# qway/nerfmeshes

Measured on AMD Instinct MI355X. Metric: rendered rays/sec (64+128 samples, 8x256 MLP), lego scene geometry, higher is better.
Workload: dtype f32; 1 GPU; nerf-synthetic lego: 8x256 coarse+fine MLP, 64 coarse + 128 fine samples, 800x800 view per step per rank, bounds [2,6], seeded weights/orbit poses; chunk_rays=65536, parallelism=single GPU

## Files before the change

### include/nerfmeshes_hip.h

```cpp
#ifndef NERFMESHES_HIP_H
#define NERFMESHES_HIP_H

#include <stdint.h>

#ifdef __cplusplus
extern "C" {
#endif

#define NM_ABI_VERSION 6

const char* nm_last_error(void);
int nm_abi_version(void);
int nm_device_count(void);

typedef struct nm_mlp_desc {
    int32_t num_layers;
    int32_t hidden_size;
    int32_t skip_step;
    int32_t num_encoding_fn_xyz;
    int32_t num_encoding_fn_dir;
    int32_t include_input_xyz;
    int32_t include_input_dir;
    int32_t use_viewdirs;
} nm_mlp_desc;
// ... 3 lines not shown
    const float* const* layers_xyz_w; const float* const* layers_xyz_b;
    const float* layers_dir0_w;       const float* layers_dir0_b;
    const float* fc_alpha_w;          const float* fc_alpha_b;
    const float* fc_rgb_w;            const float* fc_rgb_b;
    const float* fc_feat_w;           const float* fc_feat_b;
    const float* freq_xyz;
    const float* freq_dir;
} nm_mlp_weights;

typedef struct nm_mlp nm_mlp;

int nm_mlp_create(const nm_mlp_desc* desc, const nm_mlp_weights* h_weights, int device, nm_mlp** out);

enum { NM_PREC_F32 = 0, NM_PREC_BF16X3 = 1 };
enum { NM_KERNEL_GENERIC = 0x100 };
int nm_mlp_create_ex(const nm_mlp_desc* desc, const nm_mlp_weights* host_weights, int device, int precision, nm_mlp** out);
int nm_mlp_precision(const nm_mlp* mlp);
void nm_mlp_destroy(nm_mlp* mlp);
int nm_mlp_kernel_variant(const nm_mlp* mlp, int* waves_per_workgroup);
int64_t nm_mlp_flops_per_sample(const nm_mlp* mlp, int density_only);

int nm_mlp_profile_enable(int on);
int nm_mlp_profile_read(int64_t* launches, double* total_ms, double* total_flops);

int nm_mlp_sample_points(nm_mlp* mlp, const float* d_points, const float* d_dirs, int64_t n,
                         float* d_radiance, void* stream);

int nm_mlp_eval_rays(nm_mlp* mlp, const float* d_origins, int origins_per_ray, const float* d_dirs,
                     const float* d_t, int64_t rays, int32_t samples, float* d_radiance, void* stream);

int nm_mlp_grid_query(nm_mlp* mlp, const float* d_ax0, const float* d_ax1, const float* d_ax2,
                      int32_t n0, int32_t n1, int32_t n2, int64_t first, int64_t count,
                      int32_t density_only, float* d_out, void* stream);

int nm_mlp_sample_density(nm_mlp* mlp, const float* d_points, int64_t n, float* d_sigma, void* stream);

int64_t nm_mlp_density_grad_workspace_bytes(const nm_mlp* mlp, int64_t n);
int nm_mlp_density_grad(nm_mlp* mlp, const float* d_points, int64_t n, void* d_workspace, int64_t workspace_bytes,
                        float* d_grad , void* stream);


int nm_ray_bundle(const float* h_c2w, int32_t height, int32_t width, float focal, int64_t first,
                  int64_t count, float* d_dirs, float* h_origin, void* stream);

typedef struct nm_view {
    float c2w[12];
// ... 308 lines not shown
```

### nerfmeshes_amd/_lib.py

```python
import ctypes as C
import os

LIB_PATH = os.path.join(os.path.dirname(os.path.abspath(__file__)), "csrc", "libnerfmeshes_hip.so")

c_float_p = C.POINTER(C.c_float)
c_void_p = C.c_void_p


class MlpDesc(C.Structure):
    _fields_ = [(n, C.c_int32) for n in ("num_layers", "hidden_size", "skip_step", "num_encoding_fn_xyz",
                                         "num_encoding_fn_dir", "include_input_xyz", "include_input_dir",
                                         "use_viewdirs")]


class MlpWeights(C.Structure):
    _fields_ = [("layer1_w", c_void_p), ("layer1_b", c_void_p),
                ("layers_xyz_w", C.POINTER(c_void_p)), ("layers_xyz_b", C.POINTER(c_void_p)),
                ("layers_dir0_w", c_void_p), ("layers_dir0_b", c_void_p),
                ("fc_alpha_w", c_void_p), ("fc_alpha_b", c_void_p),
                ("fc_rgb_w", c_void_p), ("fc_rgb_b", c_void_p),
                ("fc_feat_w", c_void_p), ("fc_feat_b", c_void_p),
                ("freq_xyz", c_void_p), ("freq_dir", c_void_p)]


# ... 27 lines not shown

class RenderCfg(C.Structure):
    _fields_ = [("num_coarse", C.c_int32), ("num_fine", C.c_int32), ("lindisp", C.c_int32),
                ("white_background", C.c_int32), ("training", C.c_int32), ("attenuation_threshold", C.c_float)]


class View(C.Structure):
    _fields_ = [("c2w", C.c_float * 12), ("height", C.c_int32), ("width", C.c_int32), ("focal", C.c_double),
                ("use_ndc", C.c_int32), ("ndc_near", C.c_double)]


SIGNATURES = {
    "nm_last_error": (C.c_char_p, []),
    "nm_abi_version": (C.c_int, []),
    "nm_device_count": (C.c_int, []),
    "nm_mlp_create": (C.c_int, [C.POINTER(MlpDesc), C.POINTER(MlpWeights), C.c_int, C.POINTER(c_void_p)]),
    "nm_mlp_create_ex": (C.c_int, [C.POINTER(MlpDesc), C.POINTER(MlpWeights), C.c_int, C.c_int, C.POINTER(c_void_p)]),
    "nm_mlp_precision": (C.c_int, [c_void_p]),
    "nm_mlp_destroy": (None, [c_void_p]),
    "nm_mlp_kernel_variant": (C.c_int, [c_void_p, C.POINTER(C.c_int)]),
    "nm_mlp_flops_per_sample": (C.c_int64, [c_void_p, C.c_int]),
    "nm_mlp_profile_enable": (C.c_int, [C.c_int]),
    "nm_mlp_profile_read": (C.c_int, [C.POINTER(C.c_int64), C.POINTER(C.c_double), C.POINTER(C.c_double)]),
    "nm_mlp_sample_points": (C.c_int, [c_void_p, c_void_p, c_void_p, C.c_int64, c_void_p, c_void_p]),
    "nm_mlp_sample_density": (C.c_int, [c_void_p, c_void_p, C.c_int64, c_void_p, c_void_p]),
    "nm_mlp_density_grad_workspace_bytes": (C.c_int64, [c_void_p, C.c_int64]),
    "nm_mlp_density_grad": (C.c_int, [c_void_p, c_void_p, C.c_int64, c_void_p, C.c_int64, c_void_p, c_void_p]),
    "nm_mlp_eval_rays": (C.c_int, [c_void_p, c_void_p, C.c_int, c_void_p, c_void_p, C.c_int64, C.c_int32, c_void_p,
                                   c_void_p]),
    "nm_mlp_grid_query": (C.c_int, [c_void_p, c_void_p, c_void_p, c_void_p, C.c_int32, C.c_int32, C.c_int32,
                                    C.c_int64, C.c_int64, C.c_int32, c_void_p, c_void_p]),
    "nm_ray_bundle": (C.c_int, [c_float_p, C.c_int32, C.c_int32, C.c_float, C.c_int64, C.c_int64, c_void_p,
                                c_float_p, c_void_p]),
    "nm_coarse_intervals": (C.c_int, [c_void_p, c_void_p, c_void_p, C.c_int, C.c_int, C.c_int64, C.c_int32,
                                      c_void_p, c_void_p]),
    "nm_composite": (C.c_int, [c_void_p, c_void_p, c_void_p, C.c_int64, C.c_int32, C.c_float, C.c_int, C.c_int,
                               C.POINTER(BundleOut), c_void_p]),
    "nm_sample_pdf": (C.c_int, [c_void_p, c_void_p, c_void_p, C.c_int64, C.c_int32, C.c_int32, c_void_p, c_void_p]),
    "nm_render_workspace_bytes": (C.c_int64, [C.c_int64, C.c_int32, C.c_int32]),
    "nm_render_rays": (C.c_int, [c_void_p, c_void_p, C.POINTER(RenderCfg), c_void_p, C.c_int, c_void_p, c_void_p,
                                 c_void_p, C.c_int, c_void_p, c_void_p, C.c_int64, c_void_p, C.POINTER(BundleOut),
                                 C.POINTER(BundleOut), c_void_p]),
    "nm_render_view": (C.c_int, [c_void_p, c_void_p, C.POINTER(RenderCfg), C.POINTER(View), C.c_int64, C.c_int64, c_void_p,
                                 c_void_p, C.c_int, c_void_p, c_void_p, c_void_p, C.POINTER(BundleOut),
                                 C.POINTER(BundleOut), c_void_p]),
    "nm_view_rays": (C.c_int, [C.POINTER(View), C.c_int64, C.c_int64, c_void_p, c_void_p, c_void_p]),
# ... 148 lines not shown
```

### nerfmeshes_amd/csrc/mlp_api.hip

```cpp
#include <cstring>
#include <map>
#include <mutex>
#include <utility>
#include <vector>

#include "nm_internal.h"
#include "mlp_device_g.h"
#include "nerf_layerwise.h"

namespace nm {

static thread_local std::string g_error;
void set_error(const std::string& msg) { g_error = msg; }

int ensure_dynamic_lds(const void* kernel, int bytes) {
    NM_REQUIRE(bytes <= 160 * 1024, "LDS budget exceeded");
    static std::mutex lock;
    static std::map<std::pair<int, const void*>, int> have;
    int dev = 0;
    NM_HIP_CHECK(hipGetDevice(&dev));
    std::lock_guard<std::mutex> guard(lock);
    int& cur = have[{dev, kernel}];
    if (cur < bytes) {
        NM_HIP_CHECK(hipFuncSetAttribute(kernel, hipFuncAttributeMaxDynamicSharedMemorySize, bytes));
// ... 105 lines not shown
                       static_cast<float*>(m->d_blob), n, m->d_check);
    if (m->precision == NM_PREC_BF16X3) {
        const int64_t nb = (int64_t)m->b3_units * 512;
        hipLaunchKernelGGL(gather_parameters<true>, dim3((unsigned)((nb + 255) / 256)), dim3(256), 0, stream, m->d_index_b3, ptrs,
                           m->d_tmp_b3, nb, static_cast<unsigned long long*>(nullptr));
        hipLaunchKernelGGL(split_b3_kernel, dim3((unsigned)((m->b3_units * 64 + 255) / 256)), dim3(256), 0, stream,
                           m->d_tmp_b3, static_cast<uint4*>(m->d_stream_b3), (int64_t)m->b3_units);
    }
    NM_HIP_CHECK(hipGetLastError());
    ++m->refresh_count;
    return 0;
}

MlpArgs ray_mode_args(const nm_mlp* m, const float* d_origins, int origins_per_ray, const float* d_dirs, const float* d_t, int64_t rays,
                      int32_t samples, float* d_radiance) {
    MlpArgs a = m->base;
    a.mode = MODE_RAYS;
    a.a = d_origins; a.b = d_dirs; a.c = d_t;
    a.origins_per_ray = origins_per_ray; a.samples = samples;
    a.n = rays * samples; a.out = d_radiance;
    return a;
}

struct ProfRec { hipEvent_t start, stop; double flops; int slot, device; double skip_flops; };
static bool g_prof_on = false;
static std::vector<ProfRec> g_prof;
constexpr int PROF_SKIP_SLOTS = 1 << 20;
struct ProfSkips { uint32_t* d = nullptr; int used = 0; };
static std::vector<ProfSkips> g_prof_skips;

static int launch_mlp_timed(const nm_mlp* m, const MlpArgs& a, int density_only, hipStream_t stream) {
    if (!density_only && !m->desc.use_viewdirs) density_only = 2;
    auto launch = [&]() { return m->lw ? layerwise_forward(const_cast<nm_mlp*>(m), a, density_only, stream) : launch_mlp(m, a, density_only, stream); };
    if (!g_prof_on || a.n <= 0) return launch();
    ProfRec r;
    NM_HIP_CHECK(hipEventCreate(&r.start));
    NM_HIP_CHECK(hipEventCreate(&r.stop));
    r.flops = (double)a.n * (double)(density_only == 1 ? m->flops_density : m->flops_full);
    r.slot = -1; r.device = -1; r.skip_flops = 0;
    MlpArgs counted = a;
    if (a.skip_empty && !density_only && !m->lw) {
        ProfSkips* ps = m->device >= 0 && m->device < (int)g_prof_skips.size() ? &g_prof_skips[m->device] : nullptr;
        if (ps && ps->d && ps->used < PROF_SKIP_SLOTS) {
            r.slot = ps->used++; r.device = m->device;
            r.skip_flops = (double)m->plan->wg_samples * (double)(m->flops_full - m->flops_density);
            counted.skip_count = ps->d + r.slot;
        } else {
            counted.skip_empty = 0;
        }
    }
    NM_HIP_CHECK(hipEventRecord(r.start, stream));
    const int rc = m->lw ? launch() : launch_mlp(m, counted, density_only, stream);
    NM_HIP_CHECK(hipEventRecord(r.stop, stream));
    g_prof.push_back(r);
    return rc;
}

static int validate_create(const nm_mlp_desc& d, const nm_mlp_weights* w, int precision, bool force_generic) {
    NM_REQUIRE(precision == NM_PREC_F32 || precision == NM_PREC_BF16X3, "unknown precision");
    NM_REQUIRE(!force_generic || precision == NM_PREC_F32, "NM_KERNEL_GENERIC goes with NM_PREC_F32");
    NM_REQUIRE(d.use_viewdirs == 0 || d.use_viewdirs == 1, "use_viewdirs is 0 or 1");
    const bool no_view = d.use_viewdirs == 0;
    NM_REQUIRE(!no_view || precision == NM_PREC_F32, "use_viewdirs=0 networks run in fp32 only");
    NM_REQUIRE(d.num_layers >= 2 && d.num_layers <= 32, "num_layers out of range");
    NM_REQUIRE(d.skip_step >= 1, "skip_step must be >= 1");
    NM_REQUIRE(d.hidden_size >= 1 && d.num_encoding_fn_xyz >= 0 && d.num_encoding_fn_dir >= 0, "negative network dimension");
    NM_REQUIRE(no_view || d.hidden_size >= 2, "hidden_size = 1 with view directions: layers_dir[0] would have hidden_size // 2 = 0 rows");
    NM_REQUIRE(d.num_encoding_fn_xyz > 0 || d.include_input_xyz,
               "the xyz encoding is empty (num_encoding_fn_xyz = 0 without include_input_xyz): layer1 would have no input");
// ... 129 lines not shown
}

}

using namespace nm;

extern "C" {

const char* nm_last_error(void) { return g_error.c_str(); }
int nm_abi_version(void) { return NM_ABI_VERSION; }
int nm_device_count(void) {
    int n = 0;
    if (hipGetDeviceCount(&n) != hipSuccess) return -1;
    return n;
}

int nm_mlp_profile_enable(int on) {
    if (on && g_prof_skips.empty()) {
        int count = 0;
        NM_HIP_CHECK(hipGetDeviceCount(&count));
        std::vector<ProfSkips> slots(count);
        for (int dev = 0; dev < count; ++dev) {
            DeviceGuard guard(dev);
            NM_HIP_CHECK(hipMalloc(&slots[dev].d, PROF_SKIP_SLOTS * sizeof(uint32_t)));
            NM_HIP_CHECK(hipMemset(slots[dev].d, 0, PROF_SKIP_SLOTS * sizeof(uint32_t)));
        }
        g_prof_skips.swap(slots);
    }
    g_prof_on = on != 0;
    return 0;
}

int nm_mlp_profile_read(int64_t* launches, double* total_ms, double* total_flops) {
    double ms = 0, fl = 0;
    std::vector<uint32_t> skips;
    for (ProfRec& r : g_prof) {
        NM_HIP_CHECK(hipEventSynchronize(r.stop));
        float t = 0;
        NM_HIP_CHECK(hipEventElapsedTime(&t, r.start, r.stop));
        ms += t; fl += r.flops;
        (void)hipEventDestroy(r.start); (void)hipEventDestroy(r.stop);
    }
    for (int dev = 0; dev < (int)g_prof_skips.size(); ++dev) {
        ProfSkips& ps = g_prof_skips[dev];
        if (ps.used == 0) continue;
        DeviceGuard guard(dev);
        skips.resize(ps.used);
        NM_HIP_CHECK(hipMemcpy(skips.data(), ps.d, skips.size() * sizeof(uint32_t), hipMemcpyDeviceToHost));
        NM_HIP_CHECK(hipMemset(ps.d, 0, skips.size() * sizeof(uint32_t)));
        for (const ProfRec& r : g_prof)
            if (r.slot >= 0 && r.device == dev) fl -= (double)skips[r.slot] * r.skip_flops;
        ps.used = 0;
    }
    if (launches) *launches = (int64_t)g_prof.size();
    if (total_ms) *total_ms = ms;
    if (total_flops) *total_flops = fl;
    g_prof.clear();
    return 0;
}

int nm_mlp_create(const nm_mlp_desc* desc, const nm_mlp_weights* w, int device, nm_mlp** out) {
    return nm_mlp_create_ex(desc, w, device, NM_PREC_F32, out);
}

int nm_mlp_precision(const nm_mlp* m) { return m ? m->precision : -1; }

int nm_mlp_create_ex(const nm_mlp_desc* desc, const nm_mlp_weights* w, int device, int precision, nm_mlp** out) {
    NM_REQUIRE(desc && w && out, "null argument");
    const bool force_generic = (precision & NM_KERNEL_GENERIC) != 0;
    precision &= ~NM_KERNEL_GENERIC;
    const nm_mlp_desc& d = *desc;
    if (int rc = validate_create(d, w, precision, force_generic)) return rc;
    const MlpPlan* plan = nullptr;
    if (int rc = choose_plan(d, precision, force_generic, &plan)) return rc;
    LwNet* lw_net = nullptr;
    if (plan == &g_layerwise_plan) {
// ... 159 lines not shown
    return launch_mlp_timed(m, a, 0, static_cast<hipStream_t>(stream));
}

int nm_mlp_sample_density(nm_mlp* m, const float* d_points, int64_t n, float* d_sigma, void* stream) {
    NM_REQUIRE(m && d_points && d_sigma && n >= 0, "bad argument");
    NM_REQUIRE(m->precision == NM_PREC_F32, "sample_density: geometry is fp32 by contract (bf16x3 handle)");
    MlpArgs a = m->base;
    a.mode = MODE_POINTS;
    a.a = d_points; a.b = d_points; a.c = nullptr;
    a.n = n; a.out = d_sigma;
    return launch_mlp_timed(m, a, 1, static_cast<hipStream_t>(stream));
}

int nm_mlp_eval_rays(nm_mlp* m, const float* d_origins, int origins_per_ray, const float* d_dirs, const float* d_t,
                     int64_t rays, int32_t samples, float* d_radiance, void* stream) {
    NM_REQUIRE(m && d_origins && d_dirs && d_t && d_radiance && rays >= 0 && samples > 0, "bad argument");
    return launch_mlp_timed(m, ray_mode_args(m, d_origins, origins_per_ray, d_dirs, d_t, rays, samples, d_radiance), 0, static_cast<hipStream_t>(stream));
}

}

namespace nm {
int nm_mlp_eval_render_internal(nm_mlp* m, const RayGen* gen, const float* d_origins, int origins_per_ray, const float* d_dirs,
                                const float* d_t, int64_t rays, int32_t samples, float* d_radiance, hipStream_t stream) {
    NM_REQUIRE(m && (gen || (d_origins && d_dirs)) && d_t && d_radiance && rays >= 0 && samples > 0, "bad argument");
    MlpArgs a = ray_mode_args(m, d_origins, origins_per_ray, d_dirs, d_t, rays, samples, d_radiance);
    if (gen) {
        a.mode = MODE_VIEW;
        a.a = nullptr; a.b = nullptr;
        a.gen = *gen;
    }
    a.skip_empty = 1;
    return launch_mlp_timed(m, a, 0, stream);
}
}

extern "C" {

int nm_mlp_grid_query(nm_mlp* m, const float* d_ax0, const float* d_ax1, const float* d_ax2, int32_t n0, int32_t n1,
                      int32_t n2, int64_t first, int64_t count, int32_t density_only, float* d_out, void* stream) {
    NM_REQUIRE(m && d_ax0 && d_ax1 && d_ax2 && d_out, "bad argument");
    NM_REQUIRE(n0 > 0 && n1 > 0 && n2 > 0 && first >= 0 && count >= 0 &&
               first + count <= (int64_t)n0 * n1 * n2, "grid range");
    MlpArgs a = m->base;
    a.mode = MODE_GRID;
    a.a = d_ax0; a.b = d_ax1; a.c = d_ax2;
    a.n1 = n1; a.n2 = n2; a.first = first;
    a.n = count; a.out = d_out;
    return launch_mlp_timed(m, a, density_only ? 1 : 0, static_cast<hipStream_t>(stream));
}

}
```

### nerfmeshes_amd/csrc/mlp_device_r3.h

```cpp
#pragma once
#include "mlp_device.h"

namespace nm {

struct NextChunks {
    const char* s0; int b0;
    const char* s1; int b1;
};

template <int NT, int KS1, int KS2, int NW, int LDSBUF, int KCH>
__device__ __forceinline__ void gemm_stage3(f32x4 (&acc)[NT], const float (&b1)[KS1],
                                            const float (&b2)[(KS2 > 0 ? KS2 : 1)], const char* gw,
                                            const NextChunks nx, char* lds, int& slot, f32x4 (&carry)[2],
                                            int wave, int lane) {
    constexpr int KS = KS1 + KS2;
    constexpr int NCH = (KS + KCH - 1) / KCH;
    constexpr int NB = NT / 4;
    constexpr int STEP_BYTES = NT * 256;
    static_assert(NT % 4 == 0 && NB >= 1, "tile count");
    static_assert(NCH >= 2, "every stage must span at least two chunks (DMA runs two chunks ahead)");
    f32x4 ab[3];
    ab[0] = carry[0];
    ab[1] = carry[1];
#pragma unroll
// ... 60 lines not shown
    const int64_t wg_iters = mlp_wg_iters(args, NW * 16);
    auto hidden_next = [](const char* p) {
        return NextChunks{p, KCH * N::STEP, p + KCH * N::STEP, (N::KH - KCH < KCH ? N::KH - KCH : KCH) * N::STEP};
    };
    auto enc_next = [](const char* p, bool on) {
        return NextChunks{p, on ? KCH * N::STEP : 0, p + KCH * N::STEP,
                          on ? (N::EX - KCH < KCH ? N::EX - KCH : KCH) * N::STEP : 0};
    };
    auto dir_next = [](const char* p) { return NextChunks{p, KCH * N::STEPD, p + KCH * N::STEPD, KCH * N::STEPD}; };

    int slot = 0;
    f32x4 carry[2];
    if ((int64_t)blockIdx.x < wg_iters) {
        const NextChunks first = enc_next(args.wstream, true);
        stream_to_lds<NW>(first.s0, lds, first.b0, wave, lane);
        stream_to_lds<NW>(first.s1, lds + N::LDSBUF, first.b1, wave, lane);
    }
    __syncthreads();
    carry[0] = *reinterpret_cast<const f32x4*>(lds + lane * 16);
    carry[1] = *reinterpret_cast<const f32x4*>(lds + lane * 16 + 1024);

    int64_t next_it = 0;
    int turn = 0;
    for (int64_t it = blockIdx.x; it < wg_iters; it = SKIP ? next_it : it + gridDim.x) {
        bool has_next = !SKIP && it + gridDim.x < wg_iters;
        int64_t sample = (it * NW + wave) * 16 + col;
        bool valid = sample < args.n;
        if (SKIP && args.ray_tiles) {
            const uint32_t depth_slots = (uint32_t)args.samples >> 4;
            const uint32_t block = (uint32_t)it / depth_slots;
            const int64_t ray_first = ((int64_t)block * NW + wave) * args.samples;
            sample = ray_first + (((uint32_t)it - block * depth_slots) << 4) + col;
            valid = ray_first < args.n;
        }
        const int64_t sidx = valid ? sample : args.n - 1;
        const SamplePD smp = fetch_sample(args, sidx);
        const float p[3] = {smp.px, smp.py, smp.pz}, d[3] = {smp.dx, smp.dy, smp.dz};
        const float dummy[1] = {0.0f};
        float encx[N::EX];
        encode<FX, N::EX>(encx, p, args.bands_xyz, g);
        NextChunks wrap = enc_next(args.wstream, has_next);

        f32x4 acc[N::NT];
        float in[N::KH];
        const char* gw = args.wstream;
        load_bias<N::NT>(acc, lds_bias, g);
        gemm_stage3<N::NT, N::EX, 0, NW, N::LDSBUF, KCH>(acc, encx, dummy, gw, hidden_next(gw + N::EX * N::STEP), lds, slot, carry, wave, lane);
        gw += N::EX * N::STEP;
        acc_to_operand<N::NT, false>(acc, in);
        if (SKIP && threadIdx.x == 0) lds_claim[turn] = atomicAdd(args.tile_queue, 1u);

        float sigma = 0.0f;
        bool empty_tile = false;
        const int trunk_iters = density_only ? num_layers - 1 : num_layers;
#pragma unroll 1
        for (int i = 0; i < trunk_iters; ++i) {
            const bool is_feat = i == num_layers - 1;
            if (is_feat) sigma = alpha_gemv<H>(in, lds_walpha, g) + tail_bias[0];
            if (SKIP && is_feat) {
                const int epoch = (int)it + 1;
                const bool dense = valid && !(sigma <= 0.0f);
                if (dense) *lds_vote = epoch;
                __syncthreads();
                empty_tile = __builtin_amdgcn_readfirstlane(*lds_vote) != epoch;
                next_it = (int64_t)gridDim.x + (uint32_t)__builtin_amdgcn_readfirstlane((int)lds_claim[turn]);
                turn ^= 1;
                has_next = next_it < wg_iters;
                wrap = enc_next(args.wstream, has_next);
                if (empty_tile) break;
            }
            const bool skip = !is_feat && ((args.skip_mask >> i) & 1u);
            const bool last_density = density_only && i == num_layers - 2;
            load_bias<N::NT>(acc, lds_bias + H * (1 + i), g);
            {
                const char* after = gw + N::KH * N::STEP;
                NextChunks nx = hidden_next(after);
                if (skip) nx = enc_next(after, true);
                else if (is_feat) nx = dir_next(after);
                else if (last_density) nx = wrap;
                gemm_stage3<N::NT, N::KH, 0, NW, N::LDSBUF, KCH>(acc, in, dummy, gw, nx, lds, slot, carry, wave, lane);
                gw = after;
            }
            if (skip) {
                const char* after = gw + N::EX * N::STEP;
                const NextChunks nx = last_density ? wrap : hidden_next(after);
                gemm_stage3<N::NT, N::EX, 0, NW, N::LDSBUF, KCH>(acc, encx, dummy, gw, nx, lds, slot, carry, wave, lane);
                gw = after;
            }
// ... 60 lines not shown
```

### nerfmeshes_amd/csrc/nerf_mlp.hip

```cpp
#include <iterator>
#include <vector>

#include "nm_internal.h"
#include "mlp_device.h"
#include "mlp_device_r3.h"
#include "mlp_device_b3.h"
#include "mlp_device_g.h"

namespace nm {

template <int H, int FX, int FD, int NW, int KCH>
static MlpPlan make_plan() {
    return MlpPlan{H, FX, FD, NW, KCH, 0, 2 * Net<H, FX, FD, KCH>::LDSBUF, &mlp_kernel<H, FX, FD, NW, KCH, false>,
                   NW * 16, 8 / NW, &mlp_kernel<H, FX, FD, NW, KCH, false, true>, 0, nullptr, nullptr};
}

template <int H, int FX, int FD, int NW, int KCH, bool SKIP = true>
static MlpPlan make_plan3() {
    return MlpPlan{H, FX, FD, NW, KCH, 0, 3 * Net<H, FX, FD, KCH>::LDSBUF, &mlp_kernel3<H, FX, FD, NW, KCH>,
                   NW * 16, 8 / NW, &mlp_kernel3<H, FX, FD, NW, KCH, true>, 0, nullptr, nullptr,
                   SKIP ? &mlp_kernel3<H, FX, FD, NW, KCH, false, SKIP> : nullptr};
}

static const MlpPlan g_tuned_plans[] = {
// ... 51 lines not shown
    for (const MlpPlan& p : all_plans())
        if (!p.generic_nt && p.H == H && p.FX == FX && p.FD == FD) return &p;
    return nullptr;
}

const MlpPlan* find_generic_plan(int H, int L, bool long_encoding) {
    const int want = long_encoding ? G_LONG_VARIANT : 0;
    for (const MlpPlan& p : all_plans())
        if (p.generic_nt && p.variant == want && p.H >= H && forward_lds_bytes(p, H, L, 0) <= 160 * 1024) return &p;
    return nullptr;
}

int mlp_plan_info(const MlpPlan* p, int* nw) {
    *nw = p->NW;
    return p->generic_nt ? 1000 + p->generic_nt : p->variant;
}

int forward_lds_bytes(const MlpPlan& p, int H, int L, int head_floats) {
    if (p.generic_nt)
        return g_lds_bytes(p.ring_bytes, p.generic_nt, L, p.variant == G_LONG_VARIANT ? G_ENC_PARTS : 1);
    return p.ring_bytes + tuned_cache_bytes(H, L, head_floats);
}

int launch_mlp(const nm_mlp* m, const MlpArgs& args_in, int density_only, hipStream_t stream) {
    const MlpPlan* p = m->plan;
    if (args_in.n <= 0) return 0;
    MlpArgs args = args_in;
    if (!(args.skip_empty && p->kernel_skip && density_only == 0 && m->precision == NM_PREC_F32)) args.skip_empty = 0;
    args.ray_tiles = args.skip_empty && (args.mode == MODE_RAYS || args.mode == MODE_VIEW) && args.samples % 16 == 0;
    if (args.ray_tiles && mlp_wg_iters(args, p->wg_samples) > INT32_MAX) args.ray_tiles = 0;
    if (args.skip_empty && (!m->d_tile_queue || mlp_wg_iters(args, p->wg_samples) > INT32_MAX)) args.skip_empty = args.ray_tiles = 0;
    args.tile_queue = nullptr;
    if (!args.skip_empty) args.skip_count = nullptr;
    DeviceGuard guard(m->device);
    const int L = m->desc.num_layers, H = m->desc.hidden_size;
    NM_REQUIRE(density_only != 2 || (m->precision == NM_PREC_F32 && p->kernel_flat), "no kernel for use_viewdirs=0 networks in this plan");
    auto kernel = density_only == 2 ? p->kernel_flat : (args.skip_empty ? p->kernel_skip : p->kernel);
    if (m->precision == NM_PREC_BF16X3) {
        const B3Plan* b = find_b3_plan(H, m->desc.num_encoding_fn_xyz, m->desc.num_encoding_fn_dir);
        NM_REQUIRE(b && m->d_stream_b3, "no bf16x3 kernel for this network");
        const int lds_bytes = 3 * b->chunk_units * B3_UNIT + tuned_cache_bytes(H, L, 3 * H / 2 + 32);
        NM_REQUIRE(lds_bytes <= 160 * 1024, "LDS budget exceeded (bf16x3 ring + bias cache): too many layers");
        if (int rc = ensure_dynamic_lds((const void*)b->kernel, lds_bytes)) return rc;
        MlpArgs a = args;
        a.wstream = static_cast<const char*>(m->d_stream_b3);
        const unsigned grid = persistent_grid((a.n + 127) / 128, m->num_cus);
        hipLaunchKernelGGL(b->kernel, dim3(grid), dim3(512), lds_bytes, stream, a, L, density_only);
        NM_HIP_CHECK(hipGetLastError());
        return 0;
    }
    const int lds_bytes = forward_lds_bytes(*p, H, L, density_only == 2 ? 3 * H : 3 * H / 2);
    NM_REQUIRE(lds_bytes <= 160 * 1024, "LDS budget exceeded (ring + bias cache)");
    if (int rc = ensure_dynamic_lds((const void*)kernel, lds_bytes)) return rc;
    const int64_t wg_iters = mlp_wg_iters(args, p->wg_samples);
    unsigned grid = persistent_grid(wg_iters, (int64_t)m->num_cus * p->wg_per_cu);
    if (args.skip_empty) {
        const int64_t resident = (int64_t)m->num_cus * p->wg_per_cu * (p->H <= 128 ? 2 : 1);
        grid = (unsigned)(wg_iters < resident ? wg_iters : resident);
        args.tile_queue = m->d_tile_queue + (size_t)(__atomic_fetch_add(&m->tile_queue_turn, 1u, __ATOMIC_RELAXED) % TILE_QUEUE_SLOTS) * TILE_QUEUE_STRIDE;
        NM_HIP_CHECK(hipMemsetAsync(args.tile_queue, 0, sizeof(uint32_t), stream));
    }
    hipLaunchKernelGGL(kernel, dim3(grid), dim3(p->NW * 64), lds_bytes, stream, args, (int)m->desc.num_layers, density_only);
    NM_HIP_CHECK(hipGetLastError());
    return 0;
}

}
```

### nerfmeshes_amd/csrc/nm_internal.h

```cpp
#pragma once
#include <hip/hip_runtime.h>
#include <stdint.h>
#include <stdio.h>
#include <string.h>
#include <string>

#include "../../include/nerfmeshes_hip.h"
#include "mlp_pack.h"

namespace nm {

void set_error(const std::string& msg);

#define NM_HIP_CHECK(expr)                                                                   \
    do {                                                                                     \
        hipError_t _e = (expr);                                                              \
        if (_e != hipSuccess) {                                                              \
            ::nm::set_error(std::string(#expr) + ": " + hipGetErrorString(_e));              \
            return 1;                                                                        \
        }                                                                                    \
    } while (0)

#define NM_REQUIRE(cond, msg)                                                                \
    do {                                                                                     \
// ... 74 lines not shown
    int32_t samples;
    int32_t origins_per_ray;
    int32_t n1, n2;
    float* out;
    float* tape_h;
    float* tape_feat;
    float* tape_v;
    uint64_t* mask_h;
    uint64_t* mask_v;
    int64_t tiles;
    float* tape_encx;
    float* tape_encd;
    int32_t tape_v_ld;
    int32_t tape_skip_h0;
    RayGen gen;
    const void* g_tab;
    int32_t g_nsx, g_idx, g_chx;
    int32_t g_nsd, g_idd, g_chd;
    int32_t g_h, g_hd;
    int32_t skip_empty;
    int32_t ray_tiles;
    uint32_t* skip_count;
    uint32_t* tile_queue;
};

__host__ __device__ inline int64_t mlp_wg_iters(const MlpArgs& a, int wg_samples) {
    if (a.ray_tiles) {
        const int rays_per_tile = wg_samples / 16;
        return (a.n / a.samples + rays_per_tile - 1) / rays_per_tile * (a.samples / 16);
    }
    return (a.n + wg_samples - 1) / wg_samples;
}

struct MlpBwdArgs {
    const char* wstream;
    const float* walpha;
    const float* wrgb;
    const float* radiance;
    const float* grad_out;
    const uint64_t* mask_h;
    const uint64_t* mask_v;
    int64_t n, tiles;
    float* d_h;
    float* d_feat;
    float* d_v;
    float* d_last;
// ... 42 lines not shown
}

inline int tuned_cache_bytes(int H, int L, int head_floats) { return ((H * (1 + L) + H / 2 + 4 + H + head_floats) * 4 + 255) & ~255; }

int forward_lds_bytes(const MlpPlan& p, int H, int L, int head_floats);

MlpArgs ray_mode_args(const nm_mlp* m, const float* d_origins, int origins_per_ray, const float* d_dirs, const float* d_t, int64_t rays,
                      int32_t samples, float* d_radiance);

struct DwgGemmGeometry { int wa, wb, ta, tb, nba, nbb, out_pad; int64_t in_pad; };
DwgGemmGeometry dwg_gemm_geometry(int out, int64_t in);
struct DwgEpilogue { float* out; const float* bias; const float* mask; int64_t ld; int act; };
int dwg_gemm(const float* A, int out, int lda, const float* B, int64_t in, int64_t ldb, int rows, float* partial, hipStream_t stream,
             const DwgEpilogue* epilogue = nullptr);

constexpr int DW_MAX_JOBS = 16;
constexpr int HEAD_MAX_PARTS = 512;
struct DwReduceJob { const float* partial; const float* partial_bias; float* out; float* out_bias; int32_t out_ld, out_col0; };
struct DwReduceBatch { DwReduceJob job[DW_MAX_JOBS]; };
void launch_head_reduce(const float* partial, const float* partial_bias, int parts, int elems, float* out, float* out_bias,
                        hipStream_t stream);

int nm_mlp_eval_render_internal(nm_mlp* m, const RayGen* gen, const float* d_origins, int origins_per_ray, const float* d_dirs,
                                const float* d_t, int64_t rays, int32_t samples, float* d_radiance, hipStream_t stream);

}

struct nm_mlp {
    nm_mlp_desc desc;
    int device;
    const nm::MlpPlan* plan;
    void* d_blob;
    size_t blob_bytes;
    nm::MlpArgs base;
    nm::MlpBwdArgs bwd;
    int32_t* d_index;
    size_t blob_floats;
    int64_t flops_full, flops_density;
    int num_cus;
    int precision;
    void* d_stream_b3;
    float* d_tmp_b3;
    int32_t* d_index_b3;
    size_t b3_units;
    void* d_enc_tab;
    void* lw;
    unsigned long long* d_check;
// ... 6 lines not shown
```

### nerfmeshes_amd/csrc/ray_ops.hip

```cpp
#include "nm_internal.h"

namespace nm {

typedef float f32x4 __attribute__((ext_vector_type(4)));

__device__ __forceinline__ float wave_sum(float v) {
#pragma unroll
    for (int off = 32; off > 0; off >>= 1) v += __shfl_xor(v, off);
    return v;
}

__device__ __forceinline__ double shfl_up_f64(double v, int delta) {
    int lo = __double2loint(v), hi = __double2hiint(v);
    lo = __shfl_up(lo, delta);
    hi = __shfl_up(hi, delta);
    return __hiloint2double(hi, lo);
}

template <bool MUL>
__device__ __forceinline__ double wave_exclusive_scan(double v, int lane) {
    double incl = v;
#pragma unroll
    for (int off = 1; off < 64; off <<= 1) {
        const double o = shfl_up_f64(incl, off);
// ... 582 lines not shown
#define NM_COMPOSITE_BWD(P)                                                                                                     \
    hipLaunchKernelGGL(composite_backward_kernel<P>, grid, block, 0, static_cast<hipStream_t>(stream), d_radiance, d_t, d_dirs, \
                       d_noise, rays, samples, white_background, *grads, d_grad_radiance)
    switch ((samples + 63) / 64) {
        case 1: NM_COMPOSITE_BWD(1); break;
        case 2: NM_COMPOSITE_BWD(2); break;
        case 3: NM_COMPOSITE_BWD(3); break;
        case 4: NM_COMPOSITE_BWD(4); break;
        default: NM_COMPOSITE_BWD(8); break;
    }
#undef NM_COMPOSITE_BWD
    NM_HIP_CHECK(hipGetLastError());
    return 0;
}

int nm_sample_pdf_rand(const float* d_t, const float* d_weights, const float* d_u, int64_t rays, int32_t coarse,
                       int32_t fine, float* d_t_out, void* stream) {
    NM_REQUIRE(d_t && d_weights && d_u && d_t_out && rays >= 0, "bad argument");
    return launch_sample_pdf(d_t, d_weights, d_u, 1, rays, coarse, fine, d_t_out, static_cast<hipStream_t>(stream));
}

static inline size_t align256(size_t x) { return (x + 255) & ~size_t(255); }

int64_t nm_render_workspace_bytes(int64_t rays, int32_t num_coarse, int32_t num_fine) {
    const size_t sc = (size_t)num_coarse, sf = (size_t)(num_coarse + (num_fine > 0 ? num_fine : 0));
    size_t b = 0;
    b += align256(rays * sc * 4);
    b += align256(rays * sc * 16);
    b += align256(rays * sc * 4);
    if (num_fine > 0) {
        b += align256(rays * sf * 4);
        b += align256(rays * sf * 16);
    }
    return (int64_t)b;
}

static int render_impl(nm_mlp* coarse, nm_mlp* fine, const nm_render_cfg* cfg, const float* d_origins, int origins_per_ray,
                       const float* d_dirs, const RayGen* gen, const float* d_near, const float* d_far,
                       int bounds_per_ray, const float* d_u_coarse, const float* d_u_fine, int64_t rays,
                       void* d_workspace, const nm_bundle_out* coarse_out, const nm_bundle_out* fine_out,
                       hipStream_t stream) {
    if (rays <= 0) return 0;
    const int sc = cfg->num_coarse, sf = cfg->num_coarse + cfg->num_fine;
    char* ws = static_cast<char*>(d_workspace);
    float* t_c = reinterpret_cast<float*>(ws); ws += align256(rays * (size_t)sc * 4);
    float* rad_c = reinterpret_cast<float*>(ws); ws += align256(rays * (size_t)sc * 16);
    float* w_c = reinterpret_cast<float*>(ws); ws += align256(rays * (size_t)sc * 4);
    int rc;
    auto mlp = [&](nm_mlp* m, const float* t, int samples, float* rad) -> int {
        return nm_mlp_eval_render_internal(m, gen, d_origins, origins_per_ray, d_dirs, t, rays, samples, rad, stream);
    };
    if ((rc = launch_coarse_intervals(d_u_coarse, d_near, d_far, bounds_per_ray, cfg->lindisp, rays, sc, t_c, stream))) return rc;
    if ((rc = mlp(coarse, t_c, sc, rad_c))) return rc;
    nm_bundle_out co = *coarse_out;
    if (!co.d_weights) co.d_weights = w_c;
    if ((rc = launch_composite(rad_c, t_c, d_dirs, nullptr, rays, sc, cfg->attenuation_threshold, cfg->white_background,
                               cfg->training, co, stream, gen))) return rc;
    if (!fine) return 0;
    float* t_f = reinterpret_cast<float*>(ws); ws += align256(rays * (size_t)sf * 4);
    float* rad_f = reinterpret_cast<float*>(ws);
    if ((rc = launch_sample_pdf(t_c, co.d_weights, d_u_fine, 0, rays, sc, cfg->num_fine, t_f, stream))) return rc;
    if ((rc = mlp(fine, t_f, sf, rad_f))) return rc;
    return launch_composite(rad_f, t_f, d_dirs, nullptr, rays, sf, cfg->attenuation_threshold, cfg->white_background,
                            cfg->training, *fine_out, stream, gen);
}

int nm_render_rays(nm_mlp* coarse, nm_mlp* fine, const nm_render_cfg* cfg, const float* d_origins, int origins_per_ray,
                   const float* d_dirs, const float* d_near, const float* d_far, int bounds_per_ray,
                   const float* d_u_coarse, const float* d_u_fine, int64_t rays, void* d_workspace,
                   const nm_bundle_out* coarse_out, const nm_bundle_out* fine_out, void* stream_) {
    NM_REQUIRE(coarse && cfg && d_origins && d_dirs && d_near && d_far && d_u_coarse && d_workspace && coarse_out,
               "bad argument");
    NM_REQUIRE(!fine || (d_u_fine && fine_out && cfg->num_fine > 0), "fine network needs u_fine / fine_out / num_fine");
// ... 83 lines not shown
```

### nerfmeshes_amd/hip_ops.py

```python
import ctypes as C

import numpy as np
import torch

from . import _lib
from ._lib import BundleOut, MlpDesc, MlpWeights, RenderCfg, check

BUNDLE_FIELDS = ("rgb_map", "depth_map", "weights", "mask_weights", "acc_map", "disp_map")


def _ptr(t):
    return C.c_void_p(t.data_ptr()) if t is not None else C.c_void_p(None)


_raw_stream = getattr(torch._C, "_cuda_getCurrentRawStream", None)


def _stream():
    if _raw_stream is not None:
        return C.c_void_p(_raw_stream(torch.cuda.current_device()))
    return C.c_void_p(torch.cuda.current_stream().cuda_stream)


def _dev32(t, device=None, name="tensor"):
# ... 284 lines not shown
    u_coarse = _dev32(u_coarse, device)
    sc = u_coarse.numel()
    nf = 0 if fine is None else int(u_fine.numel())
    u_f = None if fine is None else _dev32(u_fine, device)
    cfg = RenderCfg(sc, nf, int(lindisp), int(white_background), int(training), float(attenuation_threshold))
    ws = _workspace(int(lib.nm_render_workspace_bytes(count, sc, nf)), device)
    ct, cout = _alloc_bundle(count, sc, device)
    ft, fout = (None, None) if fine is None else _alloc_bundle(count, sc + nf, device)
    per_ray_b = int(near.numel() == count and count > 1)
    check(lib.nm_render_view(coarse.handle, fine.handle if fine is not None else None, C.byref(cfg), C.byref(view),
                             first, count, _ptr(near), _ptr(far), per_ray_b, _ptr(u_coarse), _ptr(u_f), _ptr(ws),
                             C.byref(cout), C.byref(fout) if fout is not None else None, _stream()), "nm_render_view")
    return ct, ft


def mlp_profile_enable(on=True):
    check(_lib.load().nm_mlp_profile_enable(int(on)), "nm_mlp_profile_enable")


def mlp_profile_read():
    n, ms, fl = C.c_int64(), C.c_double(), C.c_double()
    check(_lib.load().nm_mlp_profile_read(C.byref(n), C.byref(ms), C.byref(fl)), "nm_mlp_profile_read")
    return n.value, ms.value, fl.value


def mlp_profile_read_skipped(model, samples):
    n, ms, fl = mlp_profile_read()
    full, density = model.flops_per_sample(), model.flops_per_sample(True)
    per_tile = model.kernel_variant()[1] * 16 * (full - density)
    missing = int(samples) * full - int(round(fl))
    if missing < 0 or missing % per_tile:
        raise _lib.HipLibraryError(f"profiled flops {fl!r} do not match {samples} full evaluations minus whole skipped tiles")
    return n, ms, fl, missing // per_tile


TIE_ORDERS = {"stable": 0, "reference": 1}
BUFF_REFERENCE_MAX_VOXELS = 8192


def buff_intersect(voxels, origins, dirs, near, far, samples, ids="stable"):
    if ids not in TIE_ORDERS:
        raise ValueError(f"ids must be one of {sorted(TIE_ORDERS)}, got {ids!r}")
    lib = _lib.load()
    voxels = _dev32(voxels, name="voxels")
    dev = voxels.device
    origins, dirs = _dev32(origins, dev, "origins").reshape(-1, 3), _dev32(dirs, dev, "dirs").reshape(-1, 3)
# ... 578 lines not shown
```

Before: 537,900 rays/s.

## Add early ray termination to fused MLP by skipping tiles past transmittance cutoff

Adds a per-ray-block log-transmittance table written by the fused MLP kernel. Depth tiles are reordered so that depth is the slow index, and each tile accumulates log2(1-alpha) onto the previous depth tile's value. When the next claimed tile's accumulated transmittance is below a threshold for every ray in it, the tile is marked dead: its MLP evaluation is skipped and zero radiance is written. This targets wasted MLP work behind opaque surfaces, but the depth ordering relies on cross-workgroup relaxed atomic reads, so a tile may read a predecessor's value before it is written. It also adds a memset per launch, extra workspace, and profiling counters.

```diff
diff --git a/include/nerfmeshes_hip.h b/include/nerfmeshes_hip.h
--- a/include/nerfmeshes_hip.h
+++ b/include/nerfmeshes_hip.h
@@ -49,6 +49,8 @@
 
 int nm_mlp_profile_enable(int on);
 int nm_mlp_profile_read(int64_t* launches, double* total_ms, double* total_flops);
+int nm_mlp_profile_read_tiles(int64_t* launches, double* total_ms, double* total_flops, int64_t* skipped_tiles,
+                              int64_t* terminated_tiles);
 
 int nm_mlp_sample_points(nm_mlp* mlp, const float* d_points, const float* d_dirs, int64_t n,
                          float* d_radiance, void* stream);
diff --git a/nerfmeshes_amd/_lib.py b/nerfmeshes_amd/_lib.py
--- a/nerfmeshes_amd/_lib.py
+++ b/nerfmeshes_amd/_lib.py
@@ -73,6 +73,8 @@
     "nm_mlp_flops_per_sample": (C.c_int64, [c_void_p, C.c_int]),
     "nm_mlp_profile_enable": (C.c_int, [C.c_int]),
     "nm_mlp_profile_read": (C.c_int, [C.POINTER(C.c_int64), C.POINTER(C.c_double), C.POINTER(C.c_double)]),
+    "nm_mlp_profile_read_tiles": (C.c_int, [C.POINTER(C.c_int64), C.POINTER(C.c_double), C.POINTER(C.c_double),
+                                            C.POINTER(C.c_int64), C.POINTER(C.c_int64)]),
     "nm_mlp_sample_points": (C.c_int, [c_void_p, c_void_p, c_void_p, C.c_int64, c_void_p, c_void_p]),
     "nm_mlp_sample_density": (C.c_int, [c_void_p, c_void_p, C.c_int64, c_void_p, c_void_p]),
     "nm_mlp_density_grad_workspace_bytes": (C.c_int64, [c_void_p, C.c_int64]),
diff --git a/nerfmeshes_amd/csrc/mlp_api.hip b/nerfmeshes_amd/csrc/mlp_api.hip
--- a/nerfmeshes_amd/csrc/mlp_api.hip
+++ b/nerfmeshes_amd/csrc/mlp_api.hip
@@ -151,7 +151,7 @@
     return a;
 }
 
-struct ProfRec { hipEvent_t start, stop; double flops; int slot, device; double skip_flops; };
+struct ProfRec { hipEvent_t start, stop; double flops; int slot, device; double skip_flops, dead_flops; };
 static bool g_prof_on = false;
 static std::vector<ProfRec> g_prof;
 constexpr int PROF_SKIP_SLOTS = 1 << 20;
@@ -166,14 +166,16 @@
     NM_HIP_CHECK(hipEventCreate(&r.start));
     NM_HIP_CHECK(hipEventCreate(&r.stop));
     r.flops = (double)a.n * (double)(density_only == 1 ? m->flops_density : m->flops_full);
-    r.slot = -1; r.device = -1; r.skip_flops = 0;
+    r.slot = -1; r.device = -1; r.skip_flops = 0; r.dead_flops = 0;
     MlpArgs counted = a;
     if (a.skip_empty && !density_only && !m->lw) {
         ProfSkips* ps = m->device >= 0 && m->device < (int)g_prof_skips.size() ? &g_prof_skips[m->device] : nullptr;
         if (ps && ps->d && ps->used < PROF_SKIP_SLOTS) {
             r.slot = ps->used++; r.device = m->device;
             r.skip_flops = (double)m->plan->wg_samples * (double)(m->flops_full - m->flops_density);
+            r.dead_flops = (double)m->plan->wg_samples * (double)m->flops_full;
             counted.skip_count = ps->d + r.slot;
+            counted.dead_count = ps->d + PROF_SKIP_SLOTS + r.slot;
         } else {
             counted.skip_empty = 0;
         }
@@ -349,8 +351,8 @@
         std::vector<ProfSkips> slots(count);
         for (int dev = 0; dev < count; ++dev) {
             DeviceGuard guard(dev);
-            NM_HIP_CHECK(hipMalloc(&slots[dev].d, PROF_SKIP_SLOTS * sizeof(uint32_t)));
-            NM_HIP_CHECK(hipMemset(slots[dev].d, 0, PROF_SKIP_SLOTS * sizeof(uint32_t)));
+            NM_HIP_CHECK(hipMalloc(&slots[dev].d, 2 * PROF_SKIP_SLOTS * sizeof(uint32_t)));
+            NM_HIP_CHECK(hipMemset(slots[dev].d, 0, 2 * PROF_SKIP_SLOTS * sizeof(uint32_t)));
         }
         g_prof_skips.swap(slots);
     }
@@ -359,8 +361,13 @@
 }
 
 int nm_mlp_profile_read(int64_t* launches, double* total_ms, double* total_flops) {
+    return nm_mlp_profile_read_tiles(launches, total_ms, total_flops, nullptr, nullptr);
+}
+
+int nm_mlp_profile_read_tiles(int64_t* launches, double* total_ms, double* total_flops, int64_t* skipped_tiles, int64_t* terminated_tiles) {
     double ms = 0, fl = 0;
-    std::vector<uint32_t> skips;
+    int64_t n_skipped = 0, n_dead = 0;
+    std::vector<uint32_t> skips, deads;
     for (ProfRec& r : g_prof) {
         NM_HIP_CHECK(hipEventSynchronize(r.stop));
         float t = 0;
@@ -375,10 +382,19 @@
         skips.resize(ps.used);
         NM_HIP_CHECK(hipMemcpy(skips.data(), ps.d, skips.size() * sizeof(uint32_t), hipMemcpyDeviceToHost));
         NM_HIP_CHECK(hipMemset(ps.d, 0, skips.size() * sizeof(uint32_t)));
+        deads.resize(ps.used);
+        NM_HIP_CHECK(hipMemcpy(deads.data(), ps.d + PROF_SKIP_SLOTS, deads.size() * sizeof(uint32_t), hipMemcpyDeviceToHost));
+        NM_HIP_CHECK(hipMemset(ps.d + PROF_SKIP_SLOTS, 0, deads.size() * sizeof(uint32_t)));
         for (const ProfRec& r : g_prof)
-            if (r.slot >= 0 && r.device == dev) fl -= (double)skips[r.slot] * r.skip_flops;
+            if (r.slot >= 0 && r.device == dev) {
+                fl -= (double)skips[r.slot] * r.skip_flops + (double)deads[r.slot] * r.dead_flops;
+                n_skipped += skips[r.slot];
+                n_dead += deads[r.slot];
+            }
         ps.used = 0;
     }
+    if (skipped_tiles) *skipped_tiles = n_skipped;
+    if (terminated_tiles) *terminated_tiles = n_dead;
     if (launches) *launches = (int64_t)g_prof.size();
     if (total_ms) *total_ms = ms;
     if (total_flops) *total_flops = fl;
@@ -584,7 +600,8 @@
 
 namespace nm {
 int nm_mlp_eval_render_internal(nm_mlp* m, const RayGen* gen, const float* d_origins, int origins_per_ray, const float* d_dirs,
-                                const float* d_t, int64_t rays, int32_t samples, float* d_radiance, hipStream_t stream) {
+                                const float* d_t, int64_t rays, int32_t samples, float* d_radiance, float* d_att, int64_t att_floats,
+                                hipStream_t stream) {
     NM_REQUIRE(m && (gen || (d_origins && d_dirs)) && d_t && d_radiance && rays >= 0 && samples > 0, "bad argument");
     MlpArgs a = ray_mode_args(m, d_origins, origins_per_ray, d_dirs, d_t, rays, samples, d_radiance);
     if (gen) {
@@ -593,6 +610,7 @@
         a.gen = *gen;
     }
     a.skip_empty = 1;
+    a.att = d_att; a.att_floats = d_att ? att_floats : 0;
     return launch_mlp_timed(m, a, 0, stream);
 }
 }
diff --git a/nerfmeshes_amd/csrc/mlp_device_r3.h b/nerfmeshes_amd/csrc/mlp_device_r3.h
--- a/nerfmeshes_amd/csrc/mlp_device_r3.h
+++ b/nerfmeshes_amd/csrc/mlp_device_r3.h
@@ -106,16 +106,64 @@
 
     int64_t next_it = 0;
     int turn = 0;
+    constexpr bool TERM = SKIP && H > 128;
+    const bool term = TERM && args.att != nullptr;
+    auto att_entry = [&](int64_t t, uint32_t& k) -> float* {
+        k = (uint32_t)t / args.att_blocks;
+        return args.att + ((size_t)(uint32_t)t * NW + wave);
+    };
+    bool dead = false;
+    auto claim_tile = [&](float& pre) -> uint32_t {
+        uint32_t c = 0;
+        if (lane == 0) c = atomicAdd(args.tile_queue, 1u);
+        c = (uint32_t)__builtin_amdgcn_readfirstlane((int)c);
+        pre = 0.0f;
+        if (term) {
+            const int64_t nx = (int64_t)gridDim.x + c;
+            if (nx < wg_iters && nx >= (int64_t)args.att_blocks && lane < NW)
+                pre = __hip_atomic_load(args.att + ((size_t)((uint32_t)nx - args.att_blocks) * NW + lane), __ATOMIC_RELAXED,
+                                        __HIP_MEMORY_SCOPE_AGENT);
+        }
+        return c;
+    };
+    auto claim_word = [&](uint32_t c, float pre) -> uint32_t {
+        const bool all_dead = term && __ballot(lane < NW && !(pre < -160.0f)) == 0;
+        return c | (all_dead ? 0x80000000u : 0u);
+    };
     for (int64_t it = blockIdx.x; it < wg_iters; it = SKIP ? next_it : it + gridDim.x) {
         bool has_next = !SKIP && it + gridDim.x < wg_iters;
         int64_t sample = (it * NW + wave) * 16 + col;
         bool valid = sample < args.n;
         if (SKIP && args.ray_tiles) {
             const uint32_t depth_slots = (uint32_t)args.samples >> 4;
-            const uint32_t block = (uint32_t)it / depth_slots;
+            const uint32_t div = term ? args.att_blocks : depth_slots;
+            const uint32_t q = (uint32_t)it / div, r = (uint32_t)it - q * div;
+            const uint32_t block = term ? r : q;
             const int64_t ray_first = ((int64_t)block * NW + wave) * args.samples;
-            sample = ray_first + (((uint32_t)it - block * depth_slots) << 4) + col;
+            sample = ray_first + ((term ? q : r) << 4) + col;
             valid = ray_first < args.n;
+        }
+        if (TERM && dead) {
+            if (valid && g == 0) {
+                f32x4 o4 = {0.0f, 0.0f, 0.0f, 0.0f};
+                *reinterpret_cast<f32x4*>(args.out + 4 * sample) = o4;
+            }
+            uint32_t k;
+            float* const entry = att_entry(it, k);
+            if (lane == 0) __hip_atomic_store(entry, -1e30f, __ATOMIC_RELAXED, __HIP_MEMORY_SCOPE_AGENT);
+            if (args.dead_count && threadIdx.x == 0) atomicAdd(args.dead_count, 1u);
+            if (wave == 0) {
+                float pre;
+                const uint32_t c = claim_tile(pre);
+                const uint32_t word = claim_word(c, pre);
+                if (lane == 0) lds_claim[turn] = word;
+            }
+            __syncthreads();
+            const uint32_t word = (uint32_t)__builtin_amdgcn_readfirstlane((int)lds_claim[turn]);
+            turn ^= 1;
+            next_it = (int64_t)gridDim.x + (word & 0x7fffffffu);
+            dead = (word >> 31) != 0;
+            continue;
         }
         const int64_t sidx = valid ? sample : args.n - 1;
         const SamplePD smp = fetch_sample(args, sidx);
@@ -132,7 +180,14 @@
         gemm_stage3<N::NT, N::EX, 0, NW, N::LDSBUF, KCH>(acc, encx, dummy, gw, hidden_next(gw + N::EX * N::STEP), lds, slot, carry, wave, lane);
         gw += N::EX * N::STEP;
         acc_to_operand<N::NT, false>(acc, in);
-        if (SKIP && threadIdx.x == 0) lds_claim[turn] = atomicAdd(args.tile_queue, 1u);
+        if constexpr (TERM) {
+            if (wave == 0) {
+                float pre;
+                const uint32_t claimed = claim_tile(pre);
+                const uint32_t word = claim_word(claimed, pre);
+                if (lane == 0) lds_claim[turn] = word;
+            }
+        } else if (SKIP && threadIdx.x == 0) lds_claim[turn] = atomicAdd(args.tile_queue, 1u);
 
         float sigma = 0.0f;
         bool empty_tile = false;
@@ -140,14 +195,39 @@
 #pragma unroll 1
         for (int i = 0; i < trunk_iters; ++i) {
             const bool is_feat = i == num_layers - 1;
+            float t_here = 0.0f, t_after = 0.0f, att_before = 0.0f;
+            float* entry = nullptr;
+            bool last_of_ray = false;
+            if (term && is_feat) {
+                uint32_t k;
+                entry = att_entry(it, k);
+                last_of_ray = (k << 4) + col + 1 == (uint32_t)args.samples;
+                if (valid) {
+                    t_here = args.c[sample];
+                    if (!last_of_ray) t_after = args.c[sample + 1];
+                    if (lane == 0 && k > 0)
+                        att_before = __hip_atomic_load(entry - (size_t)args.att_blocks * NW, __ATOMIC_RELAXED, __HIP_MEMORY_SCOPE_AGENT);
+                }
+            }
             if (is_feat) sigma = alpha_gemv<H>(in, lds_walpha, g) + tail_bias[0];
+            if (term && is_feat) {
+                const float dist = (last_of_ray ? 1e10f : t_after - t_here) * nm_norm3(d[0], d[1], d[2]);
+                const float a = 1.0f - expf(-(fmaxf(sigma, 0.0f) * dist));
+                float c = log2f(((1.0f - a) + 1e-10f) + 0x1p-23f) + 0x1p-8f;
+#pragma unroll
+                for (int m = 1; m < 16; m <<= 1) c += __shfl_xor(c, m);
+                if (lane == 0)
+                    __hip_atomic_store(entry, valid ? att_before + c : -1e30f, __ATOMIC_RELAXED, __HIP_MEMORY_SCOPE_AGENT);
+            }
             if (SKIP && is_feat) {
                 const int epoch = (int)it + 1;
                 const bool dense = valid && !(sigma <= 0.0f);
                 if (dense) *lds_vote = epoch;
                 __syncthreads();
                 empty_tile = __builtin_amdgcn_readfirstlane(*lds_vote) != epoch;
-                next_it = (int64_t)gridDim.x + (uint32_t)__builtin_amdgcn_readfirstlane((int)lds_claim[turn]);
+                const uint32_t word = (uint32_t)__builtin_amdgcn_readfirstlane((int)lds_claim[turn]);
+                next_it = (int64_t)gridDim.x + (word & 0x7fffffffu);
+                dead = (word >> 31) != 0;
                 turn ^= 1;
                 has_next = next_it < wg_iters;
                 wrap = enc_next(args.wstream, has_next);
diff --git a/nerfmeshes_amd/csrc/nerf_mlp.hip b/nerfmeshes_amd/csrc/nerf_mlp.hip
--- a/nerfmeshes_amd/csrc/nerf_mlp.hip
+++ b/nerfmeshes_amd/csrc/nerf_mlp.hip
@@ -1,3 +1,4 @@
+#include <cstdlib>
 #include <iterator>
 #include <vector>
 
@@ -97,6 +98,11 @@
     return p.ring_bytes + tuned_cache_bytes(H, L, head_floats);
 }
 
+static bool ray_termination_enabled() {
+    const char* e = std::getenv("NM_RAY_TERMINATION");
+    return !(e && e[0] == '0' && e[1] == 0);
+}
+
 int launch_mlp(const nm_mlp* m, const MlpArgs& args_in, int density_only, hipStream_t stream) {
     const MlpPlan* p = m->plan;
     if (args_in.n <= 0) return 0;
@@ -107,6 +113,9 @@
     if (args.skip_empty && (!m->d_tile_queue || mlp_wg_iters(args, p->wg_samples) > INT32_MAX)) args.skip_empty = args.ray_tiles = 0;
     args.tile_queue = nullptr;
     if (!args.skip_empty) args.skip_count = nullptr;
+    float* const att = args.ray_tiles ? args.att : nullptr;
+    args.att = nullptr;
+    args.att_blocks = 0;
     DeviceGuard guard(m->device);
     const int L = m->desc.num_layers, H = m->desc.hidden_size;
     NM_REQUIRE(density_only != 2 || (m->precision == NM_PREC_F32 && p->kernel_flat), "no kernel for use_viewdirs=0 networks in this plan");
@@ -134,7 +143,15 @@
         grid = (unsigned)(wg_iters < resident ? wg_iters : resident);
         args.tile_queue = m->d_tile_queue + (size_t)(__atomic_fetch_add(&m->tile_queue_turn, 1u, __ATOMIC_RELAXED) % TILE_QUEUE_SLOTS) * TILE_QUEUE_STRIDE;
         NM_HIP_CHECK(hipMemsetAsync(args.tile_queue, 0, sizeof(uint32_t), stream));
+        const int64_t depth_slots = args.samples / 16, ray_blocks = att ? wg_iters / depth_slots : 0;
+        const int64_t table = depth_slots * ray_blocks * p->NW;
+        if (att && p->H > 128 && ray_blocks >= 2 * (int64_t)grid && table <= args.att_floats && ray_termination_enabled()) {
+            args.att = att;
+            args.att_blocks = (uint32_t)ray_blocks;
+            NM_HIP_CHECK(hipMemsetAsync(att, 0, (size_t)table * sizeof(float), stream));
+        }
     }
+    if (!args.att) args.dead_count = nullptr;
     hipLaunchKernelGGL(kernel, dim3(grid), dim3(p->NW * 64), lds_bytes, stream, args, (int)m->desc.num_layers, density_only);
     NM_HIP_CHECK(hipGetLastError());
     return 0;
diff --git a/nerfmeshes_amd/csrc/nm_internal.h b/nerfmeshes_amd/csrc/nm_internal.h
--- a/nerfmeshes_amd/csrc/nm_internal.h
+++ b/nerfmeshes_amd/csrc/nm_internal.h
@@ -120,6 +120,10 @@
     int32_t ray_tiles;
     uint32_t* skip_count;
     uint32_t* tile_queue;
+    float* att;
+    int64_t att_floats;
+    uint32_t att_blocks;
+    uint32_t* dead_count;
 };
 
 __host__ __device__ inline int64_t mlp_wg_iters(const MlpArgs& a, int wg_samples) {
@@ -208,7 +212,8 @@
                         hipStream_t stream);
 
 int nm_mlp_eval_render_internal(nm_mlp* m, const RayGen* gen, const float* d_origins, int origins_per_ray, const float* d_dirs,
-                                const float* d_t, int64_t rays, int32_t samples, float* d_radiance, hipStream_t stream);
+                                const float* d_t, int64_t rays, int32_t samples, float* d_radiance, float* d_att, int64_t att_floats,
+                                hipStream_t stream);
 
 }
 
diff --git a/nerfmeshes_amd/csrc/ray_ops.hip b/nerfmeshes_amd/csrc/ray_ops.hip
--- a/nerfmeshes_amd/csrc/ray_ops.hip
+++ b/nerfmeshes_amd/csrc/ray_ops.hip
@@ -628,6 +628,8 @@
 
 static inline size_t align256(size_t x) { return (x + 255) & ~size_t(255); }
 
+static inline size_t att_table_floats(int64_t rays, int32_t samples) { return (size_t)((rays + 15) / 16 * 16) * (size_t)((samples + 15) / 16); }
+
 int64_t nm_render_workspace_bytes(int64_t rays, int32_t num_coarse, int32_t num_fine) {
     const size_t sc = (size_t)num_coarse, sf = (size_t)(num_coarse + (num_fine > 0 ? num_fine : 0));
     size_t b = 0;
@@ -638,6 +640,7 @@
         b += align256(rays * sf * 4);
         b += align256(rays * sf * 16);
     }
+    b += align256(att_table_floats(rays, (int32_t)sf) * 4);
     return (int64_t)b;
 }
 
@@ -652,9 +655,11 @@
     float* t_c = reinterpret_cast<float*>(ws); ws += align256(rays * (size_t)sc * 4);
     float* rad_c = reinterpret_cast<float*>(ws); ws += align256(rays * (size_t)sc * 16);
     float* w_c = reinterpret_cast<float*>(ws); ws += align256(rays * (size_t)sc * 4);
+    const size_t att_floats = att_table_floats(rays, fine ? sf : sc);
+    float* att = reinterpret_cast<float*>(ws + (fine ? align256(rays * (size_t)sf * 4) + align256(rays * (size_t)sf * 16) : 0));
     int rc;
     auto mlp = [&](nm_mlp* m, const float* t, int samples, float* rad) -> int {
-        return nm_mlp_eval_render_internal(m, gen, d_origins, origins_per_ray, d_dirs, t, rays, samples, rad, stream);
+        return nm_mlp_eval_render_internal(m, gen, d_origins, origins_per_ray, d_dirs, t, rays, samples, rad, att, (int64_t)att_floats, stream);
     };
     if ((rc = launch_coarse_intervals(d_u_coarse, d_near, d_far, bounds_per_ray, cfg->lindisp, rays, sc, t_c, stream))) return rc;
     if ((rc = mlp(coarse, t_c, sc, rad_c))) return rc;
diff --git a/nerfmeshes_amd/hip_ops.py b/nerfmeshes_amd/hip_ops.py
--- a/nerfmeshes_amd/hip_ops.py
+++ b/nerfmeshes_amd/hip_ops.py
@@ -330,6 +330,13 @@
     n, ms, fl = C.c_int64(), C.c_double(), C.c_double()
     check(_lib.load().nm_mlp_profile_read(C.byref(n), C.byref(ms), C.byref(fl)), "nm_mlp_profile_read")
     return n.value, ms.value, fl.value
+
+
+def mlp_profile_read_tiles():
+    n, ms, fl, sk, dead = C.c_int64(), C.c_double(), C.c_double(), C.c_int64(), C.c_int64()
+    check(_lib.load().nm_mlp_profile_read_tiles(C.byref(n), C.byref(ms), C.byref(fl), C.byref(sk), C.byref(dead)),
+          "nm_mlp_profile_read_tiles")
+    return n.value, ms.value, fl.value, sk.value, dead.value
 
 
 def mlp_profile_read_skipped(model, samples):
```

After: 658,000 rays/s, median of 6. 1.22x the previous value.
